# sevagh/demucs.cpp

Hardware: AMD Instinct MI355X
Metric: audio-sec/s (xRT) htdemucs-4s 44.1kHz stereo, ~4-min track with overlap-add (BASELINE configs[2]) (higher is better)
Workload: dtype f32 (exact bf16x3 operand split, fp32 accumulate)

## Files before the change

### demucs_cpp_amd/csrc/gemm_select.cpp

```cpp
#include "gemm_select.h"
#include <algorithm>
#include <cstdlib>

namespace dmx
{

int split_lin_mode()
{
    static const int mode = [] { const char *e = getenv("DMX_SPLIT_LIN"); return e ? atoi(e) : 1; }();
    return mode;
}

static const char *const kCfgNames[] = {"igemm_128x128", "igemm_64x64", "igemm_128x96", "igemm_128x48", "igemm_256x16", "igemm_128x32",
                                        "igemm_128x64",  "igemm_64x128", "dgemm_direct", "igemm_64x64", "igemm_64x96", "igemm_64x48",
                                        "igemm_64x32",   "igemm_64x64",  "igemm_128x16", "igemm_32x128", "igemm_32x64", "igemm_256x128", "igemm_256x128w4", "igemm_lin256x128", "igemm_256x96"};
static_assert(sizeof(kCfgNames) / sizeof(kCfgNames[0]) == kNumTileCfgs, "one label per tile configuration");

static const char *const kSplitNames[kNumTileCfgs] = {"igemm_split_128x128", nullptr, "igemm_split_128x96", "igemm_split_128x48", nullptr, "igemm_split_128x32d", "igemm_split_128x64d",
                                                      "igemm_split_64x128", nullptr, "igemm_split_64x64", "igemm_split_64x96", "igemm_split_64x48",
                                                      "igemm_split_128x32d", "igemm_split_128x64d", nullptr, "igemm_split_32x128", "igemm_split_32x64"};

static bool split_combo_exists(int cfg, int pro, int epi)
{
#define DMX_CASE(cfgid, WM_, WN_, MF, NF, PRO, EPI) case (cfgid * 100 + PRO * 10 + EPI):
    switch (cfg * 100 + pro * 10 + epi)
    {
        DMX_SPLIT_COMBOS(DMX_CASE)
        return true;
    default:
        return false;
    }
#undef DMX_CASE
}

static bool weights_exact(const std::vector<i64> *inexact, const IGemm &g)
{
    if (!inexact)
        return true;
    const i64 lo = g.w_w, hi = g.w_w + (i64)g.Np * g.Kp;
    auto it = std::lower_bound(inexact->begin(), inexact->end(), lo);
    return it == inexact->end() || *it >= hi;
}

static bool split_lin(const IGemm &g, i64 planeDelta)
{
    return gemm_is_linear(g, g.pro, g.epi, 32) && ((i64)g.B * g.xBatchStride + 64) * 4 < (1ll << 32) &&
           (planeDelta + (i64)g.Np * g.Kp + 64) * 2 < (1ll << 32);
}

static bool conv_fragments_ok(const IGemm &g)
{
    return g.Kp % 16 == 0 && g.Cin > 0 && g.Cin % 8 == 0 && g.seg0 % g.Cin == 0 && g.seg0 >= 32 && g.S1 * (g.seg0 / g.Cin) <= 32 &&
           (i64)g.S1 * g.dil1 * g.L0 * g.Cin + g.seg0 < (1ll << 31) && (g.epi != EPI_TRCONV || g.Cout % 4 == 0);
}

static constexpr double kWideMinRounds = 2.5;
static bool wide_tile_pays(const IGemm &g, i64 M, int mode)
{
    if (g.N % 256 != 0 || g.Np != g.N || g.Kp % 32 != 0 || mode == 2 || mode == 0 || (g.rowstat >= 0 && g.NB != g.N / 128))
        return false;
    if (mode == 3)
        return true;
    const i64 tm = (M + 127) / 128;
    return (double)(((tm + 7) / 8) * (g.N / 256)) / 64.0 >= kWideMinRounds;
}

static int wide_conv_width(const IGemm &g, i64 M, int mode)
{
    if (mode == 0 || mode == 2 || g.pro != PRO_NONE || !(g.epi == EPI_LINEAR || g.epi == EPI_GLU || g.epi == EPI_TRCONV) || g.rowstat >= 0)
        return 0;
    const int wnf = g.N % 256 == 0 ? 16 : g.N % 192 == 0 ? 12 : g.N == 96 ? 6 : 0;
    if (!wnf || g.Np != g.N || !conv_fragments_ok(g))
        return 0;
    if (mode == 3)
        return wnf;
    if (mode == 4 && wnf == 6)
        return 0;
    if (wnf == 6)
        return wnf;
    const i64 tm = (M + 127) / 128;
    return (double)(((tm + 7) / 8) * (g.N / (16 * wnf))) / 64.0 >= (g.N == 192 ? 0.6 : 0.9) ? wnf : 0;
}

static bool narrow_split_ok(const IGemm &g, int np)
{
    return g.pro == PRO_NONE && (g.epi == EPI_LINEAR || (g.epi == EPI_TRCONV && np == 64)) && !(g.epi == EPI_LINEAR && g.res >= 0) && g.N <= np &&
           g.Np == np && g.NB == 1 && conv_fragments_ok(g) && !(g.rowstat >= 0 && (g.epi == EPI_TRCONV || np == 64));
}

GemmChoice select_gemm(const IGemm &g, int gemm, const GemmModelFacts &m, int linMode)
{
    const i64 M = (i64)g.B * g.P1 * g.P0;
    const int cfg = g.cfg;
    if (cfg < 0 || cfg >= kNumTileCfgs)
        return GemmChoice{GF_NONE, 0, 0, "?"};
    const GemmChoice fp32{cfg == kDirectCfg ? GF_DIRECT : cfg == 19 ? GF_LIN256 : GF_TILE, 0, 0, kCfgNames[cfg]};
    if (gemm == GEMM_F32 || !m.bf16Planes || M >= (1ll << 31) - 256 || !weights_exact(m.inexactW, g))
        return fp32;
    if (cfg == 5 || cfg == 12 || cfg == 6 || cfg == 13)
    {
        const int np = (cfg == 5 || cfg == 12) ? 32 : 64;
        if (!narrow_split_ok(g, np))
            return fp32;
        return GemmChoice{GF_SPLIT_NARROW, 1, np / 16, kSplitNames[cfg]};
    }
    if (!split_combo_exists(cfg, g.pro, g.epi))
        return fp32;
    const bool planes = g.epi == EPI_KPL || g.epi == EPI_VT;
    const bool linTile = cfg == 0 || cfg == 7;
    const bool lin = split_lin(g, m.planeDelta);
    if (planes && !(linTile && lin))
        return fp32;
    if (gemm == GEMM_FP16X3 && m.fp16Plane && g.hterms && linTile && split_lin(g, 0) && weights_exact(m.inexactH, g))
        return GemmChoice{GF_SPLIT_LINH, 2, 0, cfg == 0 ? "igemm_splith_128x128" : "igemm_splith_64x128"};
    const GemmChoice wide256{GF_SPLIT_LINW, 1, 0, "igemm_split_128x256"};
    const GemmChoice linFrag{GF_SPLIT_LIN, 1, 0, kSplitNames[cfg]};
    if (planes)
        return cfg == 0 && wide_tile_pays(g, M, linMode == 0 ? 1 : linMode) ? wide256 : linFrag;
    if ((cfg == 0 || cfg == 2) && !(lin && g.epi == EPI_LINEAR && g.N % 256 == 0))
        if (const int wnf = wide_conv_width(g, M, linMode))
            return GemmChoice{GF_SPLIT_WIDE_CONV, 1, wnf, wnf == 16 ? "igemm_split_128x256" : wnf == 12 ? "igemm_split_128x192" : "igemm_split_128x96d"};
    if (!lin)
        return GemmChoice{GF_SPLIT_STAGED, 1, 0, kSplitNames[cfg]};
    if (linTile)
    {
        if (cfg == 0 && g.epi != EPI_GLU && wide_tile_pays(g, M, linMode))
            return wide256;
        if (linMode != 0)
            return linFrag;
    }
    return GemmChoice{GF_SPLIT_STAGED_LIN, 1, 0, kSplitNames[cfg]};
}

void build_chosen_plan(const PackedModel &pm, i64 seg, int B, int gemm, bool kvPlanes, const GemmModelFacts &m, int linMode, Plan &plan)
{
    PlanOpts opts;
    opts.gemm = gemm, opts.kvPlanes = kvPlanes ? 1 : 0;
    build_plan(pm, seg, B, plan, opts);
    if (kvPlanes)
        for (const Op &op : plan.ops)
            if (op.kind == OP_IGEMM && (op.g.epi == EPI_KPL || op.g.epi == EPI_VT) && select_gemm(op.g, gemm, m, linMode).arith == 0)
            {
                opts.kvPlanes = 0;
                plan = Plan();
                build_plan(pm, seg, B, plan, opts);
                break;
            }
    for (Op &op : plan.ops)
        if (op.kind == OP_IGEMM)
            op.g.choice = select_gemm(op.g, gemm, m, linMode);
}

}
```

### demucs_cpp_amd/csrc/gemm_select.h

```cpp
#pragma once
#include "plan.h"
#include <vector>

namespace dmx
{

template <class G>
inline bool gemm_is_linear(const G &a, int pro, int epi, int ktile)
{
    return pro == PRO_NONE && (epi == EPI_LINEAR || epi == EPI_SCALE_RES || epi == EPI_GLU || epi == EPI_KPL || epi == EPI_VT) && a.S1 == 1 && a.pad0 == 0 &&
           a.seg0 == a.K && a.K == a.Kp && a.K % ktile == 0 && a.Np % 4 == 0 &&
           (i64)(a.P0 - 1) * a.stride0 * a.Cin + a.seg0 <= (i64)a.L0 * a.Cin && a.P1 == a.L1 && a.stride1 == 1 && a.pad1 == 0;
}

#define DMX_SPLIT_COMBOS(X)                                                                                                   \
    X(0, 2, 2, 4, 4, PRO_NONE, EPI_LINEAR)                                                                                    \
    X(0, 2, 2, 4, 4, PRO_NONE, EPI_SCALE_RES)                                                                                 \
    X(0, 2, 2, 4, 4, PRO_NONE, EPI_GLU)                                                                                       \
    X(0, 2, 2, 4, 4, PRO_NONE, EPI_TRCONV)                                                                                    \
    X(7, 2, 2, 2, 4, PRO_NONE, EPI_LINEAR)                                                                                    \
    X(7, 2, 2, 2, 4, PRO_NONE, EPI_SCALE_RES)                                                                                 \
    X(7, 2, 2, 2, 4, PRO_NONE, EPI_GLU)                                                                                       \
    X(7, 2, 2, 2, 4, PRO_NONE, EPI_TRCONV)                                                                                    \
                              \
    X(0, 2, 2, 4, 4, PRO_NONE, EPI_KPL)                                                                                       \
    X(0, 2, 2, 4, 4, PRO_NONE, EPI_VT)                                                                                        \
    X(7, 2, 2, 2, 4, PRO_NONE, EPI_KPL)                                                                                       \
    X(7, 2, 2, 2, 4, PRO_NONE, EPI_VT)                                                                                        \
    X(2, 4, 1, 2, 6, PRO_NONE, EPI_LINEAR)                                                                                    \
    X(2, 4, 1, 2, 6, PRO_NONE, EPI_GLU)                                                                                       \
    X(2, 4, 1, 2, 6, PRO_NONE, EPI_TRCONV)                                                                                    \
         \
    X(15, 2, 2, 1, 4, PRO_NONE, EPI_LINEAR)                                                                                   \
    X(15, 2, 2, 1, 4, PRO_NONE, EPI_SCALE_RES)                                                                                \
    X(15, 2, 2, 1, 4, PRO_NONE, EPI_GLU)                                                                                      \
    X(15, 2, 2, 1, 4, PRO_NONE, EPI_TRCONV)                                                                                   \
    X(9, 2, 2, 2, 2, PRO_NONE, EPI_LINEAR)                                                                                    \
    X(9, 2, 2, 2, 2, PRO_NONE, EPI_SCALE_RES)                                                                                 \
    X(9, 2, 2, 2, 2, PRO_NONE, EPI_GLU)                                                                                       \
    X(9, 2, 2, 2, 2, PRO_NONE, EPI_TRCONV)                                                                                    \
    X(16, 2, 2, 1, 2, PRO_NONE, EPI_LINEAR)                                                                                   \
    X(16, 2, 2, 1, 2, PRO_NONE, EPI_SCALE_RES)                                                                                \
    X(16, 2, 2, 1, 2, PRO_NONE, EPI_GLU)                                                                                      \
    X(16, 2, 2, 1, 2, PRO_NONE, EPI_TRCONV)                                                                                   \
    X(10, 4, 1, 1, 6, PRO_NONE, EPI_LINEAR)                                                                                   \
    X(10, 4, 1, 1, 6, PRO_NONE, EPI_GLU)                                                                                      \
    X(10, 4, 1, 1, 6, PRO_NONE, EPI_TRCONV)                                                                                   \
                     \
    X(3, 4, 1, 2, 3, PRO_NONE, EPI_LINEAR)                                                                                    \
    X(11, 4, 1, 1, 3, PRO_NONE, EPI_LINEAR)

struct GemmModelFacts
{
    bool bf16Planes = false, fp16Plane = false;
    i64 planeDelta = 0;
    const std::vector<i64> *inexactW = nullptr, *inexactH = nullptr;
};

int split_lin_mode();

GemmChoice select_gemm(const IGemm &g, int gemm, const GemmModelFacts &m, int linMode);

void build_chosen_plan(const PackedModel &pm, i64 seg, int B, int gemm, bool kvPlanes, const GemmModelFacts &m, int linMode, Plan &plan);

inline bool operator==(const GemmChoice &a, const GemmChoice &b) { return a.family == b.family && a.arith == b.arith && a.wnf == b.wnf; }
inline bool operator!=(const GemmChoice &a, const GemmChoice &b) { return !(a == b); }

}
```

### demucs_cpp_amd/csrc/igemm_split.hip

```cpp
#include "igemm_common.h"
#include <cstdio>
#include <cstdlib>
#include <type_traits>

namespace dmx
{

__device__ __forceinline__ int swz(int row) { return (0x1320 >> (((row >> 2) & 3) * 4)) & 3; }

template <int WAVES_M, int WAVES_N, int WMF, int WNF, int PRO, int EPI, bool LIN>
__global__ __launch_bounds__(256, 2) void igemm_split_kernel(const GemmArgs p)
{
    constexpr int KT = 32;
    constexpr int BM = WAVES_M * WMF * 16;
    constexpr int BN = WAVES_N * WNF * 16;
    constexpr int LPR = 8;
    constexpr int RP = 256 / LPR;
    constexpr int AR = BM / RP;
    constexpr int BR = (BN + RP - 1) / RP;
    constexpr int BRP = BR * RP;
    static_assert(WAVES_M * WAVES_N == 4, "256 threads");
    static_assert(BM % RP == 0, "BM multiple of the staging pass");

    __shared__ u32x4 Ap0[3][BM][4], Ap1[3][BM][4];
// ... 611 lines not shown
                read_group(g + 1);
            term(g, b1[g & 1], 2);
            term(g, b2[g & 1], 1);
            if (g == (WNF == 16 ? 2 : WNF == 12 ? 1 : 0))
                split_block(other, 0);
            if (g == (WNF == 16 ? 5 : WNF == 12 ? 4 : WNF == 6 ? 2 : WNF == 4 ? 1 : 0))
                split_block(other, 1);
            term(g, b2[g & 1], 0);
            term(g, b1[g & 1], 1);
            term(g, b1[g & 1], 0);
            __builtin_amdgcn_sched_barrier(0);
        }
        asm volatile("s_waitcnt vmcnt(0)" ::: "memory");
        __syncthreads();
    };
    for (int kt = 0; kt < nk; kt += 2)
    {
        iteration(set0);
        if (kt + 1 < nk)
            iteration(set1);
    }

    if constexpr (EPI == EPI_KPL || EPI == EPI_VT)
    {
        float2(*none)[1] = nullptr;
        igemm_epilogue<1, WMF, WNF, EPI, 256>(p, acc, rowinfo_of, none, m0, n0, tileN, wave, 0, BM);
    }
    else if constexpr (WNF == 2)
    {
        float2(*rsum)[1] = reinterpret_cast<float2(*)[1]>(&Bp[0][0][0][0]);
        igemm_epilogue<1, WMF, WNF, EPI, 256>(p, acc, rowinfo_of, rsum, m0, n0, tileN, wave, 0, BM);
    }
    else if constexpr (GEN || WNF != 16)
    {
        float2(*none)[1] = nullptr;
        constexpr int JC = WNF % 4 == 0 ? 4 : 6;
#pragma unroll
        for (int jc = 0; jc < WNF; jc += JC)
        {
            f32x4 part[WMF][JC];
#pragma unroll
            for (int i = 0; i < WMF; ++i)
#pragma unroll
                for (int j = 0; j < JC; ++j)
                    part[i][j] = acc[i][jc + j];
            igemm_epilogue<1, WMF, JC, EPI, 256>(p, part, rowinfo_of, none, m0, n0 + 16 * jc, tileN, wave, 0, BM);
        }
    }
    else
    {
        static_assert(EPI == EPI_LINEAR || EPI == EPI_SCALE_RES, "plain linear layers");
        const bool hasRes = EPI == EPI_SCALE_RES || p.res != nullptr;
        const bool wantStats = p.rowstat != nullptr;
        float2(*rsum)[4] = reinterpret_cast<float2(*)[4]>(&Bp[0][0][0][0]);
#pragma unroll
        for (int jc = 0; jc < WNF; jc += 4)
        {
            float4 biasv[4], scalev[4], resv[WMF][4];
#pragma unroll
            for (int j = 0; j < 4; ++j)
            {
                const int n = n0 + (jc + j) * 16 + 4 * kq;
                biasv[j] = *reinterpret_cast<const float4 *>(p.bias + n);
                if (EPI == EPI_SCALE_RES)
                    scalev[j] = *reinterpret_cast<const float4 *>(p.scale + n);
#pragma unroll
                for (int i = 0; i < WMF; ++i)
                {
                    const i64 m = m0 + wave * (WMF * 16) + i * 16 + l15;
                    resv[i][j] = make_float4(0.f, 0.f, 0.f, 0.f);
                    if (hasRes && m < p.M)
                        resv[i][j] = *reinterpret_cast<const float4 *>(p.res + m * p.ldy + n);
                }
            }
#pragma unroll
            for (int i = 0; i < WMF; ++i)
            {
                const int rl = wave * (WMF * 16) + i * 16 + l15;
                const i64 m = m0 + rl;
                const bool rowOk = m < p.M;
                float sm = 0.f, ss = 0.f;
#pragma unroll
                for (int j = 0; j < 4; ++j)
                {
                    const int n = n0 + (jc + j) * 16 + 4 * kq;
                    const f32x4 a = acc[i][jc + j];
                    if (rowOk)
                    {
                        float4 v = make_float4(a[0] + biasv[j].x, a[1] + biasv[j].y, a[2] + biasv[j].z, a[3] + biasv[j].w);
                        if (EPI == EPI_LINEAR)
                        {
                            if (p.act)
                                v = make_float4(gelu_f(v.x), gelu_f(v.y), gelu_f(v.z), gelu_f(v.w));
                            v.x += resv[i][j].x, v.y += resv[i][j].y, v.z += resv[i][j].z, v.w += resv[i][j].w;
                        }
                        else
                            v = make_float4(resv[i][j].x + v.x * scalev[j].x, resv[i][j].y + v.y * scalev[j].y, resv[i][j].z + v.z * scalev[j].z,
                                            resv[i][j].w + v.w * scalev[j].w);
                        *reinterpret_cast<float4 *>(p.Y + m * p.ldy + n) = v;
                        sm += (v.x + v.y) + (v.z + v.w);
                        ss += (v.x * v.x + v.y * v.y) + (v.z * v.z + v.w * v.w);
                    }
                }
                if (wantStats)
                {
                    sm += __shfl_xor(sm, 16);
                    ss += __shfl_xor(ss, 16);
                    sm += __shfl_xor(sm, 32);
                    ss += __shfl_xor(ss, 32);
                    if (kq == 0)
                    {
                        rsum[rl][jc >> 2].x = sm;
                        rsum[rl][jc >> 2].y = ss;
                    }
                }
            }
        }
        if (wantStats)
        {
            __syncthreads();
            for (int e = tid; e < 2 * BM; e += 256)
            {
                const int r = e >> 1, hb = e & 1;
                const i64 m = m0 + r;
                if (m < p.M)
                {
                    float sm = 0.f, ss = 0.f;
#pragma unroll
                    for (int w = 0; w < 2; ++w)
                    {
                        sm += rsum[r][2 * hb + w].x;
                        ss += rsum[r][2 * hb + w].y;
                    }
                    float *dst = p.rowstat + (m * p.NB + 2 * tileN + hb) * 2;
                    dst[0] = sm;
                    dst[1] = ss;
                }
            }
        }
    }
}

__global__ void split3_debug_kernel(const float *x, i64 n, unsigned short *planes)
{
    const i64 i = ((i64)blockIdx.x * blockDim.x + threadIdx.x) * 2;
    if (i >= n)
        return;
    const float x0 = x[i], x1 = i + 1 < n ? x[i + 1] : 0.f;
    unsigned h1, h2, h3;
    split3_pk(x0, x1, h1, h2, h3);
    planes[i] = (unsigned short)h1, planes[n + i] = (unsigned short)h2, planes[2 * n + i] = (unsigned short)h3;
    if (i + 1 < n)
        planes[i + 1] = (unsigned short)(h1 >> 16), planes[n + i + 1] = (unsigned short)(h2 >> 16), planes[2 * n + i + 1] = (unsigned short)(h3 >> 16);
}
void launch_split3_debug(const float *d_x, i64 n, unsigned short *d_planes, hipStream_t s)
{
    const i64 pairs = (n + 1) / 2;
    hipLaunchKernelGGL(split3_debug_kernel, dim3((unsigned)((pairs + 255) / 256)), dim3(256), 0, s, d_x, n, d_planes);
}

__global__ __launch_bounds__(256) void rowscale_kernel(const GemmArgs p, float *out)
{
    const int tid = threadIdx.x, l15 = tid & 15;
    const i64 m = (i64)blockIdx.x * 16 + (tid >> 4);
    if (m >= p.M)
        return;
    const int4 ri = row_info(p, m);
    const float *row = p.X + (i64)ri.x * p.xBS + ((i64)ri.y * p.L0 + (i64)ri.z * p.stride0) * p.Cin;
    float m4[4] = {0.f, 0.f, 0.f, 0.f};
    auto take = [&](int j, int k) {
        const f32x4 v = *reinterpret_cast<const f32x4 *>(row + k);
        m4[j] = fmaxf(fmaxf(m4[j], fmaxf(fabsf(v[0]), fabsf(v[1]))), fmaxf(fabsf(v[2]), fabsf(v[3])));
    };
    int k = l15 * 4;
    for (; k + 192 < p.K; k += 256)
    {
#pragma unroll
        for (int j = 0; j < 4; ++j)
            take(j, k + 64 * j);
    }
    for (; k < p.K; k += 64)
        take(0, k);
    float mx = fmaxf(fmaxf(m4[0], m4[1]), fmaxf(m4[2], m4[3]));
#pragma unroll
    for (int off = 8; off > 0; off >>= 1)
        mx = fmaxf(mx, __shfl_xor(mx, off));
    if (l15 == 0)
        *reinterpret_cast<float2 *>(out + 2 * m) = rowscale_of(mx);
}
void launch_rowscale(const GemmArgs &a0, float *out, hipStream_t s)
{
    GemmArgs a = a0;
    a.dP0 = make_fastdiv((unsigned)a.P0), a.dP1 = make_fastdiv((unsigned)a.P1);
    hipLaunchKernelGGL(rowscale_kernel, dim3((unsigned)((a.M + 15) / 16)), dim3(256), 0, s, a, out);
}
__global__ void split3h_debug_kernel(const float *x, i64 n, float scale, unsigned short *planes)
{
    const i64 i = ((i64)blockIdx.x * blockDim.x + threadIdx.x) * 2;
    if (i >= n)
        return;
    const float x0 = x[i] * scale, x1 = (i + 1 < n ? x[i + 1] : 0.f) * scale;
    unsigned h1, h2, h3;
    split3h_pk(x0, x1, h1, h2, h3);
    planes[i] = (unsigned short)h1, planes[n + i] = (unsigned short)h2, planes[2 * n + i] = (unsigned short)h3;
    if (i + 1 < n)
        planes[i + 1] = (unsigned short)(h1 >> 16), planes[n + i + 1] = (unsigned short)(h2 >> 16), planes[2 * n + i + 1] = (unsigned short)(h3 >> 16);
}
void launch_split3h_debug(const float *d_x, i64 n, int sexp, unsigned short *d_planes, hipStream_t s)
{
    const i64 pairs = (n + 1) / 2;
    hipLaunchKernelGGL(split3h_debug_kernel, dim3((unsigned)((pairs + 255) / 256)), dim3(256), 0, s, d_x, n, ldexpf(1.0f, sexp), d_planes);
}

static dim3 grid_of(const GemmArgs &a) { return dim3(8u * ((a.tilesM + 7u) / 8u) * a.tilesN); }

static int launch_linw_conv(int wnf, GemmArgs a, hipStream_t s)
{
    a.tilesM = (unsigned)((a.M + 127) / 128);
    a.tilesN = (unsigned)((a.N + 16 * wnf - 1) / (16 * wnf));
#define DMX_LINW(WNF, EPI)                                                                                   \
    case (WNF * 10 + EPI):                                                                                   \
        hipLaunchKernelGGL((igemm_split_linw_kernel<WNF, EPI, true>), grid_of(a), dim3(256), 0, s, a); \
        return 0;
    switch (wnf * 10 + a.epi)
    {
        DMX_LINW(16, EPI_LINEAR)
        DMX_LINW(16, EPI_GLU)
        DMX_LINW(16, EPI_TRCONV)
        DMX_LINW(12, EPI_LINEAR)
        DMX_LINW(12, EPI_GLU)
        DMX_LINW(12, EPI_TRCONV)
        DMX_LINW(6, EPI_LINEAR)
        DMX_LINW(6, EPI_GLU)
        DMX_LINW(6, EPI_TRCONV)
        DMX_LINW(4, EPI_LINEAR)
        DMX_LINW(4, EPI_TRCONV)
        DMX_LINW(2, EPI_LINEAR)
    default:
        return -1;
    }
#undef DMX_LINW
}

template <int WM_, int WN_, int MF, int NF, int PRO, int EPI>
static int launch_split_one(int family, GemmArgs a, hipStream_t s)
{
    constexpr int BM = WM_ * MF * 16, BN = WN_ * NF * 16;
    constexpr bool kPlanes = EPI == EPI_KPL || EPI == EPI_VT;
    constexpr bool kLinEpi = PRO == PRO_NONE && (EPI == EPI_LINEAR || EPI == EPI_SCALE_RES || EPI == EPI_GLU);
    constexpr bool kLinTile = PRO == PRO_NONE && (kLinEpi || kPlanes) && WM_ == 2 && WN_ == 2 && NF == 4 && MF >= 2;
    a.tilesM = (unsigned)((a.M + BM - 1) / BM);
    a.tilesN = (unsigned)((a.N + BN - 1) / BN);
    switch (family)
    {
    case GF_SPLIT_STAGED:
        if constexpr (!kPlanes)
        {
            hipLaunchKernelGGL((igemm_split_kernel<WM_, WN_, MF, NF, PRO, EPI, false>), grid_of(a), dim3(256), 0, s, a);
            return 0;
        }
        break;
    case GF_SPLIT_STAGED_LIN:
        if constexpr (kLinEpi)
        {
            hipLaunchKernelGGL((igemm_split_kernel<WM_, WN_, MF, NF, PRO, EPI, true>), grid_of(a), dim3(256), 0, s, a);
            return 0;
        }
        break;
    case GF_SPLIT_LIN:
        if constexpr (kLinTile)
        {
            hipLaunchKernelGGL((igemm_split_lin_kernel<MF / 2, 8, EPI>), grid_of(a), dim3(256), 0, s, a);
            return 0;
        }
        break;
    case GF_SPLIT_LINH:
        if constexpr (kLinTile)
        {
            hipLaunchKernelGGL((igemm_split_lin_kernel<MF / 2, 8, EPI, 1>), grid_of(a), dim3(256), 0, s, a);
            return 0;
        }
        break;
    case GF_SPLIT_LINW:
        if constexpr (kLinTile && MF == 4 && EPI != EPI_GLU)
        {
            a.tilesN = (unsigned)(a.N / 256);
            hipLaunchKernelGGL((igemm_split_linw_kernel<16, EPI, false>), grid_of(a), dim3(256), 0, s, a);
            return 0;
        }
        break;
    default:
        break;
    }
    return -1;
}

int launch_igemm_split(const GemmChoice &ch, int cfg, const GemmArgs &a0, hipStream_t s)
{
    if (!a0.Wb1 || !a0.Wb2)
        return -1;
    GemmArgs a = a0;
    a.xcdMap = 1;
    a.dP0 = make_fastdiv((unsigned)a.P0), a.dP1 = make_fastdiv((unsigned)a.P1);
    if (ch.family == GF_SPLIT_WIDE_CONV || ch.family == GF_SPLIT_NARROW)
        return launch_linw_conv(ch.wnf, a, s);
#define DMX_CASE(cfgid, WM_, WN_, MF, NF, PRO, EPI) \
    case (cfgid * 100 + PRO * 10 + EPI):           \
        return launch_split_one<WM_, WN_, MF, NF, PRO, EPI>(ch.family, a, s);
    switch (cfg * 100 + a.pro * 10 + a.epi)
    {
        DMX_SPLIT_COMBOS(DMX_CASE)
    default:
        return -1;
    }
#undef DMX_CASE
}

}
```

### demucs_cpp_amd/csrc/kernels.h

```cpp
#pragma once
#include "gemm_select.h"
#include "loudness_plan.h"
#include "meters_plan.h"
#include "limiter_plan.h"
#include <hip/hip_runtime.h>
#include <cstdlib>

namespace dmx
{

struct FastDiv
{
    unsigned magic, shift;
};
inline FastDiv make_fastdiv(unsigned d)
{
    FastDiv f;
    f.magic = 0;
    f.shift = 0;
    if (d == 0)
        d = 1;
    if ((d & (d - 1)) == 0)
    {
        while ((1u << f.shift) < d)
            ++f.shift;
        return f;
    }
    unsigned s = 0;
    while ((1ull << s) < d)
        ++s;
    f.magic = (unsigned)((((unsigned long long)1 << (31 + s)) + d - 1) / d);
    f.shift = s - 1;
    return f;
}

struct GemmArgs
{
    const float *X;
    i64 xBS;
    int B, P1, P0, L1, L0, Cin;
    int S1, stride1, dil1, pad1, seg0, stride0, pad0, K, Kp;
    int pro;
    const float *proStats, *proW, *proB;
    int G0;
    const float *Wt, *bias;
    const unsigned short *Wb1, *Wb2;
    int N, Np;
    int epi, act;
    float *Y;
    i64 yBS;
    int ldy;
    const float *res, *scale, *epiStats, *epiW, *epiB;
    float *rowstat;
    int NB;
    const float *table;
    float tableScale;
    int Lout, Cout;
    int trS, trOff;
    const float *rowScale;
    unsigned short *kvPl;
    i64 kvPlane;
    int kvCol0, kvT, kvH, kvHs;
    i64 M;
    const float *zero;
    unsigned tilesM, tilesN;
    FastDiv dP0, dP1;
    int xcdMap;
};

int launch_dgemm(const GemmArgs &a, hipStream_t s, bool dry = false);

struct DconvRowArgs
{
    float *x;
    int B, T, F, C, hid;
    const float *img[2];
    float eps;
    const float *zero;
    int rowsPerXcd;
    double n1, invN1, invN1m1, n2, invN2, invN2m1;
};
int launch_dconv_row(const DconvRowArgs &a, hipStream_t s, bool dry = false);

int launch_igemm(int cfg, const GemmArgs &a, hipStream_t s, bool dry = false);
int launch_igemm_lin256(const GemmArgs &a, hipStream_t s, bool dry = false);
int launch_igemm_split(const GemmChoice &ch, int cfg, const GemmArgs &a, hipStream_t s);
void launch_rowscale(const GemmArgs &a, float *out, hipStream_t s);
void launch_split3h_debug(const float *d_x, i64 n, int sexp, unsigned short *d_planes, hipStream_t s);
void launch_split3_debug(const float *d_x, i64 n, unsigned short *d_planes, hipStream_t s);

struct ReduceArgs
{
    const float *rowstat;
    float *out;
    int B, R, NB, G0;
    double count;
    int mode;
    float eps;
    double *scratch;
    int nchunk;
};
void launch_stats_reduce(const ReduceArgs &a, hipStream_t s);

struct StftArgs
{
    const float *mix;
    float *x, *rowstat, *rowstatT;
    int B, T, seg, pad;
    const float *window, *twiddle;
};
void launch_stft(const StftArgs &a, hipStream_t s);

struct LnArgs
{
    const float *x;
    float *y;
    int rows, D, rowsPerBatch;
    const float *w, *b, *pe;
    float eps;
};
void launch_layernorm(const LnArgs &a, hipStream_t s);

struct GnArgs
{
    const float *x;
    float *y;
    const float *res;
    int B, rows, C;
    const float *stats, *w, *b;
};
void launch_gn_apply(const GnArgs &a, hipStream_t s);

struct AttnArgs
{
    const float *q, *k, *v;
    float *o;
    int ldq, ldk, ldv, ldo;
    i64 qB, kB, vB, oB;
    int B, Tq, Tk, H, hs;
    float scale;
    unsigned nQt;
    int xcdMap;
    const float *decay;
    int ldd;
    i64 dB;
    const unsigned short *kpl, *vt;
    i64 kvPlane;
    int form;
};

void launch_attention(const AttnArgs &a, hipStream_t s);
int launch_attention_split(const AttnArgs &a, hipStream_t s, bool dry = false);
int launch_attention_local(const AttnArgs &a, hipStream_t s);

struct IstftArgs
{
    const float *x, *stats;
    float *frames;
    int B, T, S;
    const float *window, *twiddle;
};
void launch_istft(const IstftArgs &a, hipStream_t s);

struct OlaArgs
{
    const float *frames, *xt, *statsT, *wss;
    float *out;
    int B, T, S, seg, pad;
};
void launch_ola(const OlaArgs &a, hipStream_t s);
struct IstftOlaArgs
{
    const float *x, *stats, *xt, *statsT, *wss, *window, *twiddle;
    float *out;
    int B, T, S, seg, pad;
    int nch, fpc;
    const float *rden;
};
void launch_istft_ola(const IstftOlaArgs &a, hipStream_t s);

struct GroupStatsArgs
{
    const float *x;
    float *out;
    double *partials;
    int B, rows, C, G;
    float eps;
};
void launch_group_stats(const GroupStatsArgs &a, hipStream_t s);
struct GnActArgs
{
    const float *x;
    float *y;
    const float *stats, *res, *w, *b, *scale;
    int B, rowsIn, C, G, mode, rowOff, rowsOut;
};
void launch_gn_act(const GnActArgs &a, hipStream_t s);
struct LstmArgs
{
    const float *xproj, *whh;
    float *out;
    void *gran;
    unsigned *status;
    int B, T, H;
};
int launch_lstm(const LstmArgs &a, hipStream_t s);
struct LocalAttnArgs
{
    const float *qkvd;
    float *out;
    int B, T, H, ld;
};
int launch_local_attn(const LocalAttnArgs &a, hipStream_t s);

struct TrackStatsTable
{
    static const int kMax = 32;
    const float *audio[kMax];
    i64 n[kMax];
    float *stats[kMax];
};
void launch_track_stats(const TrackStatsTable &t, int T, double *partials, int nblk, hipStream_t s);
void launch_track_stats_final(const TrackStatsTable &t, int T, const double *partials, int nblk, hipStream_t s);
void launch_track_stats(const float *audio, i64 n, double *partials, int nblk, hipStream_t s);
void launch_track_stats_final(const double *partials, int nblk, i64 n, float *stats, hipStream_t s);
struct TrackSegItem
{
    const float *audio;
    const float *stats;
    i64 n;
    int shift;
    int seg;
};
struct TrackSegIdx
{
    static const int kMax = 64;
    TrackSegItem v[kMax];
};
void launch_track_gather(const TrackSegItem *items, int nIdx, i64 seg, i64 stride, float *mixes, hipStream_t s);
void launch_track_gather(const float *audio, i64 n, const float *stats, int shiftOffset, i64 seg, i64 stride,
                         i64 len, const int *segIdx, int nIdx, float *mixes, hipStream_t s);
struct TrackOlaEntry
{
    const float *segOut;
    const float *stats;
    float *out;
    i64 n, len, i0, i1;
    i64 gBase, slot0;
    int nSeg, shift;
};
struct TrackOlaTable
{
    static const int kMax = 32;
    TrackOlaEntry e[kMax];
};
void launch_track_ola(const TrackOlaEntry *entries, int T, int S, i64 seg, i64 stride, i64 ring, int layout, int planeBase,
                      int nPlanes, hipStream_t s);
void launch_track_ola(const float *segOut, int nSeg, int S, i64 seg, i64 stride, i64 len, i64 n, int shiftOffset,
                      const float *stats, float *out, int layout, int planeBase, int nPlanes, i64 i0, i64 i1, hipStream_t s,
                      int gBase = 0);
struct TrackEnsPiece
{
    const float *stats;
    float *out;
    i64 n, i0, i1;
    i64 itemLo, slotLo;
    int nMin, nTail;
};
struct TrackEnsCopy
{
    int shift, nseg;
};
struct TrackEnsTable
{
    static const int kMaxPieces = 16, kMaxCopies = 256;
    static const int kMaxTail = 2048;
    TrackEnsPiece p[kMaxPieces];
    TrackEnsCopy c[kMaxCopies];
};
void launch_track_ola_ens(const TrackEnsPiece *pieces, const TrackEnsCopy *copies, int P, int N, const float *segOut, int S,
                          i64 seg, i64 stride, i64 ring, int layout, int planeBase, int nPlanes, hipStream_t s);
struct TrackBagPiece
{
    const float *stats;
    float *out;
    i64 n, i0, i1;
};
struct TrackBagModel
{
    int itemLo, slotLo;
    int nMin, nTail;
};
struct TrackBagTable
{
    static const int kMaxPieces = 8, kMaxModels = 32, kMaxCopies = 256, kMaxBag = 8, kMaxStems = 8;
    static const int kMaxTail = 12288;
    TrackBagPiece p[kMaxPieces];
    TrackBagModel m[kMaxModels];
    TrackEnsCopy c[kMaxCopies];
    float w[kMaxBag * kMaxStems];
    const float *ring[kMaxBag];
    i64 ringBlocks[kMaxBag];
};
i64 track_ola_bag_tail_entries(const TrackBagModel *models, int P, int Q, int N, int S, const float *w);
bool launch_track_ola_bag(const TrackBagPiece *pieces, const TrackBagModel *models, const TrackEnsCopy *copies, int P, int Q, int N,
                          const float *w, const float *const *rings, const i64 *ringBlocks, int S, i64 seg, i64 stride, int layout,
                          int planeBase, int nPlanes, hipStream_t s);
struct PcmPiece
{
    const float *planes;
    unsigned char *pcm;
    unsigned *peaks;
    i64 n, planeStride, outStride, i0, i1;
};
struct PcmTable
{
    static const int kMax = 32;
    PcmPiece p[kMax];
};
void launch_pcm_peak(const PcmPiece *pieces, int P, int S, int stem, hipStream_t s);
void launch_pcm_encode(const PcmPiece *pieces, int P, int S, int stem, int encoding, int clip, hipStream_t s);
struct PcmGains
{
    static const int kMaxOut = 8, kMaxSrc = 7;
    float g[kMaxOut][kMaxSrc];
    int nOut, S;
};
struct RemixPiece : PcmPiece
{
    const float *mix;
};
struct RemixTable
{
    static const int kMax = 32;
    RemixPiece p[kMax];
};
void launch_remix_peak(const RemixPiece *pieces, int P, const PcmGains &G, hipStream_t s);
void launch_remix_encode(const RemixPiece *pieces, int P, const PcmGains &G, int encoding, int clip, hipStream_t s);
struct LoudPiece : RemixPiece
{
    const float *gains;
};
struct LoudTable
{
    static const int kMax = 32;
    LoudPiece p[kMax];
};
void launch_loud_encode(const LoudPiece *pieces, int P, const PcmGains &G, int encoding, int clip, hipStream_t s);
void launch_loud_measure(const RemixPiece &pc, const PcmGains &G, const LoudPlan &lp, unsigned char *work, int slot0, double *eOut,
                         void *resOut, hipStream_t s, hipEvent_t *marks = nullptr);
void launch_loud_gain(const unsigned char *work, i64 slotBytes, int nOut, unsigned *peaks, int mode, int targetC, float maxPeak,
                      const float *table, float *gains, void *report, hipStream_t s);
void launch_loud_gain_tp(const unsigned char *work, i64 slotBytes, int nOut, unsigned *peaks, const unsigned *tp, int mode, int targetC,
                         float maxPeak, const float *table, float *gains, void *report, hipStream_t s);
void launch_true_peak(const RemixPiece *pieces, int P, const PcmGains &G, const TpFilter &f, hipStream_t s);
void launch_meters(const unsigned char *work, int slot0, int nSignals, const LoudPlan &lp, const unsigned *tp, void *out, hipStream_t s);
struct LimJob
{
    RemixPiece pc;
    PcmGains G;
    const float *gains;
    float gainImm, ceiling;
    int qa, qr, link;
    unsigned char *work;
    const int32_t *tables;
    void *res;
};
void launch_limit(const LimJob &job, const TpFilter &f, bool truePeak, hipStream_t s, hipEvent_t *marks = nullptr);
struct LimitPiece : LoudPiece
{
    const float *gplane;
    i64 gplaneStride;
};
struct LimitTable
{
    static const int kMax = 32;
    LimitPiece p[kMax];
};
void launch_limit_encode(const LimitPiece *pieces, int P, const PcmGains &G, int encoding, int clip, hipStream_t s);
struct ResamplePiece
{
    const float *src;
    float *dst;
    i64 n, dstStem, dstChan, dstStep, k0, k1;
};
struct ResampleTable
{
    static const int kMax = 32;
    ResamplePiece p[kMax];
// ... 48 lines not shown
```

### demucs_cpp_amd/csrc/plan.h

```cpp
#pragma once
#include <cstdint>
#include <string>
#include <vector>

namespace dmx
{
typedef int64_t i64;
static inline int rup(int v, int m) { return (v + m - 1) / m * m; }

enum OpKind
{
    OP_IGEMM = 0,
    OP_STATS_REDUCE,
    OP_STFT,
    OP_LAYERNORM,
    OP_GN_APPLY,
    OP_ATTENTION,
    OP_ISTFT,
    OP_OLA,
    OP_TAP,
    OP_GROUP_STATS,
    OP_GN_ACT,
    OP_LSTM,
    OP_LOCAL_ATTN,
    OP_DCONV_ROW,
};

enum Prologue
{
    PRO_NONE = 0,
    PRO_AFFINE = 1,
    PRO_GN_GELU = 2,
};

enum Epilogue
{
    EPI_LINEAR = 0,
    EPI_SCALE_RES = 1,
    EPI_GLU = 2,
    EPI_GN_GLU_SCALE_RES = 3,
    EPI_STATS_ONLY = 4,
    EPI_TRCONV = 5,
    EPI_STATS_FACT = 6,
    EPI_KPL = 7,
    EPI_VT = 8,
};

enum StatsMode
{
    MODE_RSTD = 0,
    MODE_ZNORM = 1,
};

enum GemmFamily
{
    GF_NONE = 0,
    GF_DIRECT,
    GF_TILE,
    GF_LIN256,
    GF_SPLIT_STAGED,
    GF_SPLIT_STAGED_LIN,
    GF_SPLIT_LIN,
    GF_SPLIT_LINH,
    GF_SPLIT_LINW,
    GF_SPLIT_WIDE_CONV,
    GF_SPLIT_NARROW,
};
struct GemmChoice
{
    int family;
    int arith;
    int wnf;
    const char *label;
};

struct IGemm
{
    int B, P1, P0;
    i64 x, xBatchStride;
    int L1, L0, Cin;
    int S1, stride1, dil1, pad1;
    int seg0, stride0, pad0;
    int K;
    int Kp;
    int pro;
    i64 proStats;
    i64 proW_w, proB_w;
    int G0;
    i64 w_w;
    i64 bias_w;
    int N, Np;
    int epi, act;
    i64 y, yBatchStride;
    int ldy;
    i64 res;
    i64 scale_w;
    i64 epiStats;
    i64 epiW_w, epiB_w;
    i64 rowstat;
    int NB;
    i64 table_w;
    float tableScale;
    int Lout, Cout;
    int trS, trOff;
    int cfg;
    GemmChoice choice;
    i64 kv;
    int kvCol0, kvT, kvH, kvHs;
    int hterms = 0;
};

struct StatsReduce
{
    i64 rowstat;
    i64 out;
    int B, R;
    int NB;
    int G0;
    double count;
    int mode;
    float eps;
    i64 scratch;
    int nchunk;
};

struct Stft
{
    i64 mix;
    i64 x;
    i64 rowstat;
    i64 rowstatT;
    int B, T, seg, pad;
    i64 window, twiddle;
};

struct LayerNorm
{
    i64 x, y;
    int rows, D, rowsPerBatch;
    i64 w_w, b_w;
    i64 pe;
    float eps;
};

struct GnApply
{
    i64 x, y, res;
    int B, rows, C;
    i64 stats;
    i64 w_w, b_w;
};

struct Attention
{
    i64 q, k, v, o;
    int ldq, ldk, ldv, ldo;
    i64 qBatch, kBatch, vBatch, oBatch;
    int B, Tq, Tk, H, hs;
    float scale;
    int split;
    i64 kpl = -1, vt = -1;
    int form = 0;
};

struct Istft
{
    i64 x;
    i64 stats;
    i64 frames;
    int B, T, S;
    i64 window, twiddle;
    int fused;
};

struct Ola
{
    i64 frames;
    i64 xt;
    i64 statsT;
    i64 wss;
    i64 out;
    int B, T, S, seg, pad;
    i64 x, stats, window, twiddle;
    i64 rden;
};

struct GroupStats
{
    i64 x;
    i64 out;
    int B, rows, C, G;
    float eps;
    i64 scratch;
};
struct GnAct
{
    i64 x, y, stats, res;
    i64 w_w, b_w, scale_w;
    int B, rowsIn, C, G, mode, rowOff, rowsOut;
};
struct Lstm
{
    i64 xproj;
    i64 whh_w;
    i64 out;
    i64 sync;
    int B, T, H;
};
i64 lstm_sync_floats(int B, int H);
i64 lstm_xchg_floats(int B, int T, int H);
struct LocalAttn
{
    i64 qkvd;
    i64 out;
    int B, T, H, ld;
};

struct DconvRow
{
    i64 x;
    int B, T, F, C, hid;
    i64 k1_w[2], k1_b[2], gn1_w[2], gn1_b[2], k2_w[2], k2_b[2], k2f_w[2], k2f_b[2], gn2_w[2], gn2_b[2], scale_w[2];
    i64 img_w[2];
    float eps;
};
struct DconvRowGeo
{
    int HP, RPL, NP, WS, nWp, oW3, oLf, oCst, nWk;
    bool resident;
};
bool dconv_row_geo(int C, int hid, DconvRowGeo &g);
i64 dconv_row_image_floats(int C, int hid);
size_t dconv_row_lds_bytes(int C, int hid, int T);

struct Tap
{
    i64 off;
    int shape[4];
    i64 batchStride;
};

struct Op
{
    int kind;
    int stream;
    int waitOp = -1;
    bool signals = false;
    std::string name;
    IGemm g;
    StatsReduce sr;
    Stft stft;
    LayerNorm ln;
    GnApply gn;
    Attention at;
    Istft istft;
    Ola ola;
    Tap tap;
    GroupStats gs;
    GnAct ga;
    Lstm lstm;
    LocalAttn la;
    DconvRow dr;
};

struct Geo
{
    i64 seg, le, pad, pad_end, padded, nfr;
    i64 Lt[5];
};
Geo make_geo(i64 seg);

struct PackedModel
{
    int arch = 4;
    int n_sources = 4;
    int dim = 512;
    int n_tensors = 0;
    std::vector<float> blob;
    std::vector<std::pair<std::string, i64>> index;
    i64 find(const std::string &name) const;
    bool has(const std::string &name) const;
};

struct TileCfg
{
    int BM, BN;
};
static const TileCfg kTileCfgs[] = {
    {128, 128},
    {64, 64},
    {128, 96},
    {128, 48},
    {256, 16},
    {128, 32},
    {128, 64},
    {64, 128},
    {16, 256},
    {64, 64},
    {64, 96},
    {64, 48},
    {64, 32},
    {64, 64},
    {128, 16},
    {32, 128},
    {32, 64},
    {256, 128},
    {256, 128},
    {256, 128},
    {256, 96},
};
static const int kNumTileCfgs = 21;
static const int kDirectCfg = 8;
int half_cfg(int cfg, bool stat);
int refine_cfg(int cfg, i64 M, int N, bool stat);
bool lin256_shape(const IGemm &g);
bool shortk_shape(const IGemm &g);
bool direct_available(int N, int S1, int seg0, int pro, int epi);
int choose_cfg(i64 M1, int N, bool paired);

enum GemmMode
{
    GEMM_F32 = 0,
    GEMM_BF16X3 = 1,
    GEMM_FP16X3 = 2,
};
struct PlanOpts
{
    int gemm = GEMM_F32;
    int kvPlanes = 0;
};

struct Plan
{
    int B = 1;
    int gemm = GEMM_F32;
    Geo geo;
    int S = 4, D = 512;
    i64 arenaFloats = 0;
    std::vector<float> constants;
    std::vector<Op> ops;
    i64 zeroOff = 0;
    i64 mixOff = 0;
    i64 outOff = 0;
};

bool load_and_pack(const std::string &path, PackedModel &pm, std::string &err);
void build_plan(const PackedModel &pm, i64 seg, int B, Plan &plan, const PlanOpts &opts = PlanOpts());
void build_plan_v3(const PackedModel &pm, i64 seg, int B, Plan &plan, const PlanOpts &opts = PlanOpts());
struct Range
{
    i64 lo, hi;
};
void op_access(const Op &op, std::vector<Range> &reads, std::vector<Range> &writes);
void compute_deps(Plan &plan);

}
```

### demucs_cpp_amd/csrc/plan_describe.h

```cpp
#pragma once
#include "attention_select.h"
#include "plan.h"
#include <algorithm>
#include <cstdio>
#include <string>

namespace dmx
{
inline std::string describe_choice(const IGemm &g)
{
    char t[256];
    snprintf(t, sizeof(t), "cfg=%d family=%d arith=%d wnf=%d label=%s BM=%d BN=%d NB=%d", g.cfg, g.choice.family, g.choice.arith, g.choice.wnf,
             g.choice.label ? g.choice.label : "-", kTileCfgs[g.cfg].BM, kTileCfgs[g.cfg].BN, g.NB);
    return t;
}

inline std::string describe_op(const Op &op)
{
    std::vector<Range> rd, wr, scr;
    op_access(op, rd, wr);
    if (op.kind == OP_STATS_REDUCE && op.sr.scratch >= 0)
        scr.push_back(Range{op.sr.scratch, op.sr.scratch + (i64)op.sr.B * op.sr.nchunk * 4});
    if (op.kind == OP_GROUP_STATS && op.gs.scratch >= 0)
        scr.push_back(Range{op.gs.scratch, op.gs.scratch + (i64)op.gs.B * op.gs.G * 32 * 4});
    if (op.kind == OP_LSTM && op.lstm.sync >= 0)
        scr.push_back(Range{op.lstm.sync, op.lstm.sync + lstm_xchg_floats(op.lstm.B, op.lstm.T, op.lstm.H)});
    std::string all = "name=" + op.name + " kind=" + std::to_string(op.kind) + " stream=" + std::to_string(op.stream);
    const std::vector<Range> *lists[3] = {&rd, &wr, &scr};
    const char *keys[3] = {" reads=", " writes=", " scratch="};
    for (int k = 0; k < 3; ++k)
    {
        all += keys[k];
        for (const Range &r : *lists[k])
            all += std::to_string(r.lo) + ":" + std::to_string(r.hi) + ",";
    }
    auto word = [&](const char *k, i64 v) { all += std::string(" ") + k + "=" + std::to_string(v); };
    switch (op.kind)
    {
    case OP_IGEMM:
    {
        const IGemm &g = op.g;
        const i64 M = (i64)g.B * g.P1 * g.P0;
        word("K", g.K), word("N", g.N), word("M", M), word("pro", g.pro), word("epi", g.epi), word("act", g.act), word("res", g.res >= 0);
        word("stat", g.rowstat >= 0), word("hterms", g.hterms);
        word("y", g.y), word("ldy", g.ldy), word("Kp", g.Kp), word("w_w", g.w_w), word("bias_w", g.bias_w), word("kvCol0", g.kvCol0);
        all += " " + describe_choice(g);
        if (g.rowstat >= 0)
            all += " rowstat=" + std::to_string(g.rowstat) + ":" + std::to_string(g.rowstat + M * std::max(g.NB, 1) * 2);
        if (g.kv >= 0)
            word("kv", g.kv), word("kvPlane", (i64)g.B * g.kvT * g.kvH * g.kvHs);
        break;
    }
    case OP_ATTENTION:
        all += std::string(" label=") + (op.at.split ? "attention_split" : "attention");
        word("K", op.at.hs), word("T", op.at.Tk), word("split", op.at.split), word("planes", op.at.kpl >= 0);
        word("Tq", op.at.Tq), word("H", op.at.H), word("B", op.at.B);
        all += std::string(" form=") + att_form_name(op.at.form);
        {
            char sc[32];
            snprintf(sc, sizeof(sc), " scale=%.9g", (double)op.at.scale);
            all += sc;
        }
        if (op.at.kpl >= 0)
            word("kpl", op.at.kpl), word("vt", op.at.vt), word("kvPlane", (i64)op.at.B * op.at.Tk * op.at.H * op.at.hs);
        break;
    case OP_STATS_REDUCE: all += " label=stats_reduce", word("K", (i64)op.sr.R * op.sr.NB); break;
    case OP_STFT: all += " label=stft", word("K", 4096); break;
    case OP_LAYERNORM: all += " label=layernorm", word("K", op.ln.D); break;
    case OP_GN_APPLY: all += " label=gn_apply"; break;
    case OP_ISTFT: all += " label=istft", word("K", 4096), word("fused", op.istft.fused); break;
    case OP_OLA: all += op.ola.x >= 0 ? " label=istft_ola" : " label=ola", word("K", 4096), word("fused", op.ola.x >= 0); break;
    case OP_GROUP_STATS: all += " label=group_stats", word("K", (i64)op.gs.rows * (op.gs.C / op.gs.G)); break;
    case OP_GN_ACT: all += " label=gn_act", word("mode", op.ga.mode); break;
    case OP_LSTM: all += " label=lstm", word("K", op.lstm.H), word("T", op.lstm.T); break;
    case OP_LOCAL_ATTN: all += " label=local_attn", word("K", op.la.H / 4), word("T", op.la.T); break;
    case OP_DCONV_ROW: all += " label=dconv_row", word("K", 3 * op.dr.C), word("T", op.dr.T), word("H", op.dr.hid); break;
    default: all += " label=tap"; break;
    }
    return all;
}
}
```

Before: 3069.

## Add persistent streaming split-GEMM kernel for narrow GLU/TRCONV conv shapes

Adds a persistent kernel for wide-conv split bf16x3 GEMMs with N of 96 or 192 and small K. Each workgroup loads the whole weight panel into LDS once, then streams several M tiles per XCD. It double-buffers the A loads and the bf16 splits so they overlap the MFMA work. The selector turns it on only when enough M tiles exist per XCD slot, which cuts repeated weight loads and launch/tail overhead but adds register and LDS pressure and a new code path.

```diff
diff --git a/demucs_cpp_amd/csrc/gemm_select.cpp b/demucs_cpp_amd/csrc/gemm_select.cpp
--- a/demucs_cpp_amd/csrc/gemm_select.cpp
+++ b/demucs_cpp_amd/csrc/gemm_select.cpp
@@ -82,6 +82,29 @@
     return (double)(((tm + 7) / 8) * (g.N / (16 * wnf))) / 64.0 >= (g.N == 192 ? 0.6 : 0.9) ? wnf : 0;
 }
 
+#ifndef DMX_STREAM_MIN_ROUNDS
+#define DMX_STREAM_MIN_ROUNDS 3.5
+#endif
+static constexpr double kStreamMinRounds = DMX_STREAM_MIN_ROUNDS;
+bool stream_shape_ok(const IGemm &g, int wnf)
+{
+    const int nk = (g.Kp + 31) / 32;
+    if (!(wnf == 6 || wnf == 12) || g.N != 16 * wnf || g.Np != g.N || g.pro != PRO_NONE || g.rowstat >= 0 || !conv_fragments_ok(g))
+        return false;
+    if (wnf == 6)
+        return (g.epi == EPI_GLU && (nk == 2 || nk == 5)) || (g.epi == EPI_TRCONV && nk == 3);
+    return g.epi == EPI_GLU && nk == 3;
+}
+static bool stream_pays(const IGemm &g, i64 M, int wnf, int mode)
+{
+    if ((mode != 1 && mode != 6) || !stream_shape_ok(g, wnf))
+        return false;
+    if (mode == 6)
+        return true;
+    const i64 perXcd = ((M + 127) / 128 + 7) / 8;
+    return (double)perXcd / (32.0 * stream_wgs_per_cu(wnf, (g.Kp + 31) / 32)) >= kStreamMinRounds;
+}
+
 static bool narrow_split_ok(const IGemm &g, int np)
 {
     return g.pro == PRO_NONE && (g.epi == EPI_LINEAR || (g.epi == EPI_TRCONV && np == 64)) && !(g.epi == EPI_LINEAR && g.res >= 0) && g.N <= np &&
@@ -119,7 +142,8 @@
         return cfg == 0 && wide_tile_pays(g, M, linMode == 0 ? 1 : linMode) ? wide256 : linFrag;
     if ((cfg == 0 || cfg == 2) && !(lin && g.epi == EPI_LINEAR && g.N % 256 == 0))
         if (const int wnf = wide_conv_width(g, M, linMode))
-            return GemmChoice{GF_SPLIT_WIDE_CONV, 1, wnf, wnf == 16 ? "igemm_split_128x256" : wnf == 12 ? "igemm_split_128x192" : "igemm_split_128x96d"};
+            return GemmChoice{GF_SPLIT_WIDE_CONV, 1, wnf, wnf == 16 ? "igemm_split_128x256" : wnf == 12 ? "igemm_split_128x192" : "igemm_split_128x96d",
+                              stream_pays(g, M, wnf, linMode) ? 1 : 0};
     if (!lin)
         return GemmChoice{GF_SPLIT_STAGED, 1, 0, kSplitNames[cfg]};
     if (linTile)
diff --git a/demucs_cpp_amd/csrc/gemm_select.h b/demucs_cpp_amd/csrc/gemm_select.h
--- a/demucs_cpp_amd/csrc/gemm_select.h
+++ b/demucs_cpp_amd/csrc/gemm_select.h
@@ -63,7 +63,10 @@
 
 void build_chosen_plan(const PackedModel &pm, i64 seg, int B, int gemm, bool kvPlanes, const GemmModelFacts &m, int linMode, Plan &plan);
 
-inline bool operator==(const GemmChoice &a, const GemmChoice &b) { return a.family == b.family && a.arith == b.arith && a.wnf == b.wnf; }
+constexpr int stream_wgs_per_cu(int wnf, int nk) { return nk * 2 * 16 * wnf * 64 * 2 <= 160 * 1024 ? 2 : 1; }
+bool stream_shape_ok(const IGemm &g, int wnf);
+
+inline bool operator==(const GemmChoice &a, const GemmChoice &b) { return a.family == b.family && a.arith == b.arith && a.wnf == b.wnf && a.stream == b.stream; }
 inline bool operator!=(const GemmChoice &a, const GemmChoice &b) { return !(a == b); }
 
 }
diff --git a/demucs_cpp_amd/csrc/igemm_split.hip b/demucs_cpp_amd/csrc/igemm_split.hip
--- a/demucs_cpp_amd/csrc/igemm_split.hip
+++ b/demucs_cpp_amd/csrc/igemm_split.hip
@@ -937,6 +937,8 @@
     GemmArgs a = a0;
     a.xcdMap = 1;
     a.dP0 = make_fastdiv((unsigned)a.P0), a.dP1 = make_fastdiv((unsigned)a.P1);
+    if (ch.stream)
+        return ch.family == GF_SPLIT_WIDE_CONV ? launch_igemm_split_stream(ch.wnf, a, s) : -1;
     if (ch.family == GF_SPLIT_WIDE_CONV || ch.family == GF_SPLIT_NARROW)
         return launch_linw_conv(ch.wnf, a, s);
 #define DMX_CASE(cfgid, WM_, WN_, MF, NF, PRO, EPI) \
diff --git a/demucs_cpp_amd/csrc/igemm_stream.hip b/demucs_cpp_amd/csrc/igemm_stream.hip
--- /dev/null
+++ b/demucs_cpp_amd/csrc/igemm_stream.hip
@@ -0,0 +1,273 @@
+#include "igemm_common.h"
+#include <type_traits>
+
+namespace dmx
+{
+
+__device__ __forceinline__ int swz_s(int row) { return (0x1320 >> (((row >> 2) & 3) * 4)) & 3; }
+
+template <int U, int END, class F>
+__device__ __forceinline__ bool steps_until(F &&f)
+{
+    if constexpr (U < END)
+    {
+        if (!f(std::integral_constant<int, U>{}))
+            return false;
+        return steps_until<U + 1, END>(f);
+    }
+    return true;
+}
+
+template <int WNF, int NK, int EPI>
+__global__ __launch_bounds__(256, stream_wgs_per_cu(WNF, NK)) void igemm_split_stream_kernel(const GemmArgs p)
+{
+    constexpr int KT = 32, WMF = 2, BM = 128, BN = 16 * WNF, NG = WNF / 2;
+    constexpr int PW = WNF / 2;
+    static_assert(WNF == 6 || WNF == 12, "N = 96 / 192");
+    static_assert(NK >= 2 && NK * 2 * BN * 64 <= 80 * 1024, "two workgroups per CU at least");
+    __shared__ u32x4 Bp[NK][2][BN][4];
+
+    const int tid = threadIdx.x, lane = tid & 63, wave = tid >> 6;
+    const int l15 = lane & 15, kq = lane >> 4;
+    const unsigned xcd = blockIdx.x & 7u, wj = blockIdx.x >> 3;
+    const unsigned t0 = wj * p.streamRun * 8u + xcd;
+    if (t0 >= p.tilesM)
+        return;
+    const int nb = (int)min(p.streamRun, (p.tilesM - t0 + 7u) / 8u);
+
+    const int rowLenI = p.L0 * p.Cin;
+    const float *aRow[WMF];
+    unsigned aMask[WMF];
+    int gS1, gOffb, gTapC, gTapOff, lb = 0, lkt = 0;
+    auto begin_block = [&](int r) {
+        const i64 rowLen = (i64)p.L0 * p.Cin;
+        const i64 mb = ((i64)t0 + 8 * (i64)r) * BM + wave * (WMF * 16);
+#pragma unroll
+        for (int i = 0; i < WMF; ++i)
+        {
+            const i64 m = min(mb + i * 16 + l15, p.M - 1);
+            const int4 ri = row_info(p, m);
+            const int taps0 = p.seg0 / p.Cin;
+            const int in1_0 = ri.y * p.stride1 - p.pad1;
+            const int e0 = (ri.z * p.stride0 - p.pad0) * p.Cin;
+            aRow[i] = p.X + (i64)ri.x * p.xBS + (i64)in1_0 * rowLen + e0;
+            aMask[i] = 0;
+            unsigned m0bits = 0;
+            for (int t = 0; t < taps0; ++t)
+            {
+                const int e = e0 + t * p.Cin;
+                m0bits |= (e >= 0 && e < rowLenI ? 1u : 0u) << t;
+            }
+            for (int s = 0; s < p.S1; ++s)
+            {
+                const int in1 = in1_0 + s * p.dil1;
+                if (in1 >= 0 && in1 < p.L1)
+                    aMask[i] |= m0bits << (s * taps0);
+            }
+        }
+        gS1 = 0, gOffb = kq * 8, gTapC = 0, gTapOff = kq * 8;
+        if (p.S1 > 1)
+            while (gOffb >= p.seg0)
+            {
+                gOffb -= p.seg0;
+                ++gS1;
+            }
+        while (gTapOff >= p.Cin)
+        {
+            gTapOff -= p.Cin;
+            ++gTapC;
+        }
+    };
+
+    f32x4 aRaw[2][WMF][2];
+    u32x4 aPl[2][WMF][3];
+    auto load_A = [&](auto setTag) {
+        constexpr int SET = decltype(setTag)::value;
+        const unsigned tapBit = gTapC < 32 ? 1u << gTapC : 0u;
+        const int segOff = gS1 * p.dil1 * rowLenI + gOffb;
+#pragma unroll
+        for (int i = 0; i < WMF; ++i)
+        {
+            const float *src = (aMask[i] & tapBit) ? aRow[i] + segOff : p.zero;
+            aRaw[SET][i][0] = *reinterpret_cast<const f32x4 *>(src);
+            aRaw[SET][i][1] = *reinterpret_cast<const f32x4 *>(src + 4);
+        }
+        if (++lkt == NK)
+        {
+            lkt = 0;
+            begin_block(++lb);
+            return;
+        }
+        gOffb += KT;
+        if (p.S1 > 1 && gOffb >= p.seg0)
+        {
+            gOffb -= p.seg0;
+            ++gS1;
+        }
+        gTapOff += KT;
+        while (gTapOff >= p.Cin)
+        {
+            gTapOff -= p.Cin;
+            ++gTapC;
+        }
+    };
+    auto split_block = [&](auto setTag, int i) {
+        constexpr int SET = decltype(setTag)::value;
+        const f32x4 lo = aRaw[SET][i][0], hi = aRaw[SET][i][1];
+        unsigned h1[4], h2[4], h3[4];
+        split3_pk(lo[0], lo[1], h1[0], h2[0], h3[0]);
+        split3_pk(lo[2], lo[3], h1[1], h2[1], h3[1]);
+        split3_pk(hi[0], hi[1], h1[2], h2[2], h3[2]);
+        split3_pk(hi[2], hi[3], h1[3], h2[3], h3[3]);
+        u32x4 q1{h1[0], h1[1], h1[2], h1[3]}, q2{h2[0], h2[1], h2[2], h2[3]}, q3{h3[0], h3[1], h3[2], h3[3]};
+        asm volatile("" : "+v"(q1), "+v"(q2), "+v"(q3));
+        aPl[SET][i][0] = q1;
+        aPl[SET][i][1] = q2;
+        aPl[SET][i][2] = q3;
+    };
+
+    const std::integral_constant<int, 0> set0{};
+    const std::integral_constant<int, 1> set1{};
+    begin_block(0);
+    load_A(set0);
+    load_A(set1);
+
+    {
+        const int wv = __builtin_amdgcn_readfirstlane(wave);
+        const unsigned bVoff = ((unsigned)(lane >> 2) * (unsigned)p.Kp + 8u * (unsigned)((lane & 3) ^ swz_s(lane >> 2))) * 2u;
+#pragma unroll
+        for (int kt = 0; kt < NK; ++kt)
+#pragma unroll
+            for (int i = 0; i < PW; ++i)
+            {
+                const int c = wv * PW + i, pl = c / WNF, cb = c % WNF;
+                const char *src = reinterpret_cast<const char *>(pl ? p.Wb2 : p.Wb1) + (size_t)(16 * cb) * (size_t)p.Kp * 2u + bVoff + kt * (KT * 2);
+                u32x4 *dst = &Bp[kt][pl][16 * cb][0];
+                if (((kt * 2 + pl) * BN + 16 * cb) * 64 + 1024 <= 65536)
+                    load_to_lds_b128(reinterpret_cast<const float *>(src), reinterpret_cast<float4 *>(dst));
+                else
+                    dst[lane] = *reinterpret_cast<const u32x4 *>(src);
+            }
+    }
+    split_block(set0, 0);
+    split_block(set0, 1);
+    asm volatile("s_waitcnt vmcnt(0) lgkmcnt(0)" ::: "memory");
+    __syncthreads();
+    load_A(set0);
+
+    constexpr int JC = WNF % 4 == 0 ? 4 : 6;
+    f32x4 acc[WNF / JC][WMF][JC];
+#pragma unroll
+    for (int c = 0; c < WNF / JC; ++c)
+#pragma unroll
+        for (int i = 0; i < WMF; ++i)
+#pragma unroll
+            for (int j = 0; j < JC; ++j)
+                acc[c][i][j] = f32x4{0.f, 0.f, 0.f, 0.f};
+
+    const int fslot = kq ^ swz_s(l15);
+    int cb = 0;
+    auto step = [&](auto uTag) -> bool {
+        constexpr int U = decltype(uTag)::value, PAR = U & 1, kt = U % NK;
+        const std::integral_constant<int, PAR ^ 1> other{};
+        u32x4 b1[2][2], b2[2][2];
+        auto read_group = [&](int g) {
+#pragma unroll
+            for (int u = 0; u < 2; ++u)
+            {
+                const int r = (2 * g + u) * 16 + l15;
+                b1[g & 1][u] = Bp[kt][0][r][fslot];
+                b2[g & 1][u] = Bp[kt][1][r][fslot];
+            }
+        };
+        auto term = [&](int g, u32x4(&b)[2], int plane) {
+#pragma unroll
+            for (int i = 0; i < WMF; ++i)
+#pragma unroll
+                for (int u = 0; u < 2; ++u)
+                {
+                    f32x4 &d = acc[(2 * g + u) / JC][i][(2 * g + u) % JC];
+                    d = __builtin_amdgcn_mfma_f32_16x16x32_bf16(__builtin_bit_cast(bf16x8, b[u]), __builtin_bit_cast(bf16x8, aPl[PAR][i][plane]), d, 0, 0, 0);
+                }
+        };
+        constexpr bool AHEAD = WNF <= 6;
+        if (AHEAD)
+            read_group(0);
+#pragma unroll
+        for (int g = 0; g < NG; ++g)
+        {
+            if (!AHEAD)
+                read_group(g);
+            else if (g + 1 < NG)
+                read_group(g + 1);
+            term(g, b1[g & 1], 2);
+            term(g, b2[g & 1], 1);
+            if (kt != NK - 1 && g == 0)
+                split_block(other, 0);
+            if (kt != NK - 1 && g == 1)
+            {
+                split_block(other, 1);
+                load_A(other);
+            }
+            term(g, b2[g & 1], 0);
+            term(g, b1[g & 1], 1);
+            term(g, b1[g & 1], 0);
+            __builtin_amdgcn_sched_barrier(0);
+        }
+        if constexpr (kt == NK - 1)
+        {
+            const i64 m0 = ((i64)t0 + 8 * (i64)cb) * BM;
+            auto rowinfo_of = [&](int r) -> int4 { return row_info(p, m0 + r); };
+            float2(*none)[1] = nullptr;
+#pragma unroll
+            for (int c = 0; c < WNF / JC; ++c)
+            {
+                int n0 = 16 * JC * c;
+                asm volatile("" : "+s"(n0));
+                igemm_epilogue<1, WMF, JC, EPI, 256>(p, acc[c], rowinfo_of, none, m0, n0, 0u, wave, 0, BM);
+#pragma unroll
+                for (int i = 0; i < WMF; ++i)
+#pragma unroll
+                    for (int j = 0; j < JC; ++j)
+                        acc[c][i][j] = f32x4{0.f, 0.f, 0.f, 0.f};
+            }
+            split_block(other, 0);
+            split_block(other, 1);
+            load_A(other);
+            return ++cb < nb;
+        }
+        return true;
+    };
+    constexpr int PERIOD = NK % 2 == 0 ? NK : 2 * NK;
+    while (steps_until<0, PERIOD>(step))
+    {
+    }
+}
+
+int launch_igemm_split_stream(int wnf, GemmArgs a, hipStream_t s)
+{
+    a.tilesM = (unsigned)((a.M + 127) / 128);
+    a.tilesN = 1;
+    const int nk = (a.Kp + 31) >> 5;
+    if (a.N != 16 * wnf || a.Np != a.N || a.pro != PRO_NONE || a.rowstat || (a.epi == EPI_LINEAR && a.res))
+        return -1;
+    const unsigned perXcd = (a.tilesM + 7u) / 8u, slots = 32u * (unsigned)stream_wgs_per_cu(wnf, nk);
+    a.streamRun = (perXcd + slots - 1u) / slots;
+    const dim3 grid(8u * ((perXcd + a.streamRun - 1u) / a.streamRun));
+#define DMX_STREAM(WNF, NK, EPI)                                                                         \
+    case ((WNF * 10 + NK) * 10 + EPI):                                                                   \
+        hipLaunchKernelGGL((igemm_split_stream_kernel<WNF, NK, EPI>), grid, dim3(256), 0, s, a); \
+        return 0;
+    switch ((wnf * 10 + nk) * 10 + a.epi)
+    {
+        DMX_STREAM(6, 2, EPI_GLU)
+        DMX_STREAM(6, 5, EPI_GLU)
+        DMX_STREAM(6, 3, EPI_TRCONV)
+        DMX_STREAM(12, 3, EPI_GLU)
+    default:
+        return -1;
+    }
+#undef DMX_STREAM
+}
+
+}
diff --git a/demucs_cpp_amd/csrc/kernels.h b/demucs_cpp_amd/csrc/kernels.h
--- a/demucs_cpp_amd/csrc/kernels.h
+++ b/demucs_cpp_amd/csrc/kernels.h
@@ -66,6 +66,7 @@
     unsigned tilesM, tilesN;
     FastDiv dP0, dP1;
     int xcdMap;
+    unsigned streamRun;
 };
 
 int launch_dgemm(const GemmArgs &a, hipStream_t s, bool dry = false);
@@ -85,6 +86,7 @@
 int launch_igemm(int cfg, const GemmArgs &a, hipStream_t s, bool dry = false);
 int launch_igemm_lin256(const GemmArgs &a, hipStream_t s, bool dry = false);
 int launch_igemm_split(const GemmChoice &ch, int cfg, const GemmArgs &a, hipStream_t s);
+int launch_igemm_split_stream(int wnf, GemmArgs a, hipStream_t s);
 void launch_rowscale(const GemmArgs &a, float *out, hipStream_t s);
 void launch_split3h_debug(const float *d_x, i64 n, int sexp, unsigned short *d_planes, hipStream_t s);
 void launch_split3_debug(const float *d_x, i64 n, unsigned short *d_planes, hipStream_t s);
diff --git a/demucs_cpp_amd/csrc/plan.h b/demucs_cpp_amd/csrc/plan.h
--- a/demucs_cpp_amd/csrc/plan.h
+++ b/demucs_cpp_amd/csrc/plan.h
@@ -72,6 +72,7 @@
     int arith;
     int wnf;
     const char *label;
+    int stream;
 };
 
 struct IGemm
diff --git a/demucs_cpp_amd/csrc/plan_describe.h b/demucs_cpp_amd/csrc/plan_describe.h
--- a/demucs_cpp_amd/csrc/plan_describe.h
+++ b/demucs_cpp_amd/csrc/plan_describe.h
@@ -10,8 +10,8 @@
 inline std::string describe_choice(const IGemm &g)
 {
     char t[256];
-    snprintf(t, sizeof(t), "cfg=%d family=%d arith=%d wnf=%d label=%s BM=%d BN=%d NB=%d", g.cfg, g.choice.family, g.choice.arith, g.choice.wnf,
-             g.choice.label ? g.choice.label : "-", kTileCfgs[g.cfg].BM, kTileCfgs[g.cfg].BN, g.NB);
+    snprintf(t, sizeof(t), "cfg=%d family=%d arith=%d wnf=%d label=%s BM=%d BN=%d NB=%d streaming=%d", g.cfg, g.choice.family, g.choice.arith, g.choice.wnf,
+             g.choice.label ? g.choice.label : "-", kTileCfgs[g.cfg].BM, kTileCfgs[g.cfg].BN, g.NB, g.choice.stream);
     return t;
 }
 
```

New measurement: 3085 (median of 6 runs). No clear change (+0.5%).
